# vliu15/speech-masters-thesis

Measured on AMD Instinct MI355X. Metric: LJSpeech utterances/sec per VQ-VAE train step, higher is better.
Workload: dtype bf16

## Files before the change

speech-masters-thesis_amd/csrc/conv_ws.hip:

```cpp
#include <algorithm>
#include <cstdlib>
#include <type_traits>

#include "smt_common.h"
#include "conv_common.h"

namespace smt {

#ifndef SMT_WS_STAMP
#define SMT_WS_STAMP 0
#endif
#if SMT_WS_STAMP
__device__ unsigned long long ws_dbg[256 * 8 * 8];
#define WS_T(var) const unsigned long long var = __builtin_readcyclecounter()
#define WS_ACC(k, a, b) do { if (lane == 0 && wg < 256) ws_dbg[(wg * 8 + wave) * 8 + (k)] += (b) - (a); } while (0)
#else
#define WS_T(var) do {} while (0)
#define WS_ACC(k, a, b) do {} while (0)
#endif
constexpr int WS_AGPR_TAPS = 8;
constexpr int WS_BM = 128, WS_BN = 128, WS_NT = 256, WS_EPI = 128 * 256;
constexpr int WS_KC = 128, WS_ROWB = WS_KC * 2, WS_KSTEPS = WS_KC / 16;

template <int I, int N, typename F>
__device__ __forceinline__ void static_for(F&& f) {
  if constexpr (I < N) {
    f(std::integral_constant<int, I>{});
    static_for<I + 1, N>(f);
  }
}


__device__ __forceinline__ bf16x8 ws_wfrag(const unsigned char* wrow, int kk, int hh, int co) {
  return *reinterpret_cast<const bf16x8*>(wrow + (((2 * kk + hh) ^ (co & 15)) << 4));
}

__device__ __forceinline__ void ws_decode(int tiles_per_batch, int rs, int tile, int& b, int& cls, int& t0) {
  const int bb = tile / tiles_per_batch;
  b = bb / rs; cls = bb - b * rs;
  t0 = (tile - bb * tiles_per_batch) * WS_BM;
}

__device__ __forceinline__ unsigned ws_tap_base(unsigned abase, int ar, int hh) { return abase + ar * WS_ROWB + ((hh ^ swz256_row(ar)) << 4); }
template <int NTAPS>
__device__ __forceinline__ unsigned ws_frag_addr(const unsigned (&tap_base)[NTAPS], int q) {
  return tap_base[q / WS_KSTEPS] ^ (32u * (q % WS_KSTEPS));
}

template <int MW>
__device__ __forceinline__ void ws_read_frags(bf16x8 (&afr)[MW], unsigned ap) {
#pragma unroll
  for (int i = 0; i < MW; ++i)
    asm volatile("ds_read_b128 %0, %1 offset:%2" : "=v"(afr[i]) : "v"(ap), "n"(i * 32 * WS_ROWB));
}
__device__ __forceinline__ void ws_first_use(f32x16& acc) { asm volatile("s_nop 4" : "+v"(acc)); }
__device__ __forceinline__ void ws_first_use(f32x16& acc0, f32x16& acc1) { asm volatile("s_nop 4" : "+v"(acc0), "+v"(acc1)); }
__device__ __forceinline__ void ws_mfma(f32x16& acc, const bf16x8& w, const bf16x8& a, bool w_in_agpr) {
  if (w_in_agpr) asm volatile("v_mfma_f32_32x32x16_bf16 %0, %1, %2, %0" : "+v"(acc) : "a"(w), "v"(a));
  else asm volatile("v_mfma_f32_32x32x16_bf16 %0, %1, %2, %0" : "+v"(acc) : "v"(w), "v"(a));
}
template <int MW>
__device__ __forceinline__ void ws_drain(f32x16 (&acc)[MW]) {
  static_assert(MW == 2 || MW == 4, "the drain names two or four accumulators");
#define WS_DRAIN_NOPS "s_nop 15\n\ts_nop 15\n\ts_nop 15\n\ts_nop 15"
  if constexpr (MW == 4) asm volatile(WS_DRAIN_NOPS : "+v"(acc[0]), "+v"(acc[1]), "+v"(acc[2]), "+v"(acc[3]));
  else asm volatile(WS_DRAIN_NOPS : "+v"(acc[0]), "+v"(acc[1]));
#undef WS_DRAIN_NOPS
}

template <int NTAPS, int MODE>
__global__ __launch_bounds__(WS_NT) void conv_ws_kernel(ConvArgs p, const __bf16* __restrict__ zero_page,
                                                        int tiles_per_wg, int buf_bytes) {
  const bool has_y = MODE == 0 ? (p.y != nullptr) : (MODE == 2);
  const bool has_act_out = MODE == 0 ? (p.act_out != 0) : (MODE == 1);
  const bool has_res = MODE == 0 ? (p.res != nullptr) : (MODE == 2);
  const bool has_epi_act = MODE == 0 ? (p.epi_act != 0) : (MODE == 2);
  typedef __bf16 T;
  constexpr int BM = WS_BM, BN = WS_BN, KC = WS_KC, NT = WS_NT, MW = BM / 32, ROWB = WS_ROWB;
  extern __shared__ __attribute__((aligned(1024))) unsigned char smem[];
  const int tid = threadIdx.x, lane = tid & 63, wave = tid >> 6;
  const int r = lane & 31, hh = lane >> 5;
  const int lrow = lane >> 4, lch = lane & 15;
  const int n0 = blockIdx.y * BN;
  const int rs = p.rs;

  int wg, tile_begin, tile_end;
  if (!wg_tile_run(p.tiles_per_batch * p.B * rs, tiles_per_wg, wg, tile_begin, tile_end)) return;

  unsigned char* lds_res = smem + 2 * (size_t)buf_bytes + wave * (WS_EPI / 4);
  unsigned char* lds_act = lds_res + WS_EPI;
  const unsigned lds_base = (unsigned)(uintptr_t)(__attribute__((address_space(3))) unsigned char*)smem;

  bf16x8 wfrag[NTAPS][KC / 16];
  {
    const int co = n0 + wave * 32 + r;
#pragma unroll
    for (int s = 0; s < NTAPS; ++s) {
      const unsigned char* wrow = reinterpret_cast<const unsigned char*>(p.w) + ((size_t)s * p.Cout + co) * ROWB;
#pragma unroll
      for (int kk = 0; kk < KC / 16; ++kk)
        wfrag[s][kk] = ws_wfrag(wrow, kk, hh, co);
    }
  }
  const int col0 = n0 + wave * 32 + 4 * hh;
  float bval[16];
#pragma unroll
  for (int e = 0; e < 16; ++e) bval[e] = p.bias ? p.bias[col0 + 8 * (e >> 2) + (e & 3)] : 0.f;
  const int rows_in = BM + (NTAPS - 1) * p.dil;
  const int rows_pad = (rows_in + 3) & ~3;

  auto decode = [&](int tile, int& b, int& cls, int& t0) { ws_decode(p.tiles_per_batch, rs, tile, b, cls, t0); };
  const unsigned pitch_x = (unsigned)p.ldx * rs * 2u;
  const unsigned voff_a0 = (unsigned)(4 * wave + lrow) * pitch_x + (unsigned)((lch ^ swz256_row(4 * wave + lrow)) << 4);
  const int ngroups = rows_pad >> 2;
  auto stage_a = [&](int tile, int buf) {
    int b, cls, t0;
    decode(tile, b, cls, t0);
    const int len_full = p.lens_in ? min(scalar_load_i32(p.lens_in + b), p.Tin) : p.Tin;
    const int len_in = max(0, (len_full - cls + rs - 1) / rs);
    const __amdgpu_buffer_rsrc_t rx = ws_rsrc(p.x, ((long long)b * p.x_bs + (long long)cls * p.ldx) * 2, (unsigned)len_in * pitch_x);
    unsigned vo = voff_a0 + (unsigned)(t0 - p.pad) * pitch_x;
    unsigned char* dst = smem + (size_t)buf * buf_bytes + wave * 1024;
    for (int g = wave; g < ngroups; g += NT / 64) {
      ws_dma16(rx, vo, dst);
      vo += 16u * pitch_x; dst += 4096;
    }
  };
  const unsigned echunk = (unsigned)(((lane & 3) ^ ((lane >> 4) & 3)) << 4);
  auto stage_epi = [&](const void* base, long long bs, int ld, int b, int cls, int t0, int Tc, unsigned char* dst) {
    const unsigned pitch = (unsigned)ld * rs * 2u;
    const __amdgpu_buffer_rsrc_t re = ws_rsrc(base, ((long long)b * bs + (long long)cls * ld + n0 + wave * 32) * 2, (unsigned)Tc * pitch);
    unsigned vo = (unsigned)(t0 + (lane >> 2)) * pitch + echunk;
#pragma unroll
    for (int q = 0; q < BM / 16; ++q) {
      ws_dma16(re, vo, dst + q * 1024);
      vo += 16u * pitch;
    }
  };

  stage_a(tile_begin, 0);
  vm_wait<0>();
  for (int tile = tile_begin; tile < tile_end; ++tile) {
    const int buf = (tile - tile_begin) & 1;
    int b, cls, t0;
    decode(tile, b, cls, t0);
    const int Tc = (p.Tout - cls + rs - 1) / rs;
    WS_T(c0);
    __syncthreads();
    WS_T(c1);
    __amdgpu_buffer_rsrc_t rx_n = ws_rsrc(p.x, 0, 0), re_res = rx_n, re_act = rx_n;
    unsigned vo_in = 0, vo_res = 0, vo_act = 0, pitch_res = 0, pitch_act = 0;
    int n_in = 0;
    const int wave_s = __builtin_amdgcn_readfirstlane(wave);
    if constexpr (MODE == 2) {
      if (tile + 1 < tile_end) {
        int nb, ncls, nt0;
        decode(tile + 1, nb, ncls, nt0);
        const int len_full = p.lens_in ? min(scalar_load_i32(p.lens_in + nb), p.Tin) : p.Tin;
        const int len_in = max(0, (len_full - ncls + rs - 1) / rs);
        rx_n = ws_rsrc(p.x, ((long long)nb * p.x_bs + (long long)ncls * p.ldx) * 2, (unsigned)len_in * pitch_x);
        vo_in = voff_a0 + (unsigned)(nt0 - p.pad) * pitch_x;
        n_in = ngroups;
      }
      pitch_res = (unsigned)p.ldr * rs * 2u; pitch_act = (unsigned)p.ldgh * rs * 2u;
      re_res = ws_rsrc(p.res, ((long long)b * p.res_bs + (long long)cls * p.ldr + n0 + wave_s * 32) * 2, (unsigned)Tc * pitch_res);
      re_act = ws_rsrc(p.gate_h, ((long long)b * p.gh_bs + (long long)cls * p.ldgh + n0 + wave_s * 32) * 2, (unsigned)Tc * pitch_act);
      vo_res = (unsigned)(t0 + (lane >> 2)) * pitch_res + echunk;
      vo_act = (unsigned)(t0 + (lane >> 2)) * pitch_act + echunk;
    } else {
      if (tile + 1 < tile_end) stage_a(tile + 1, buf ^ 1);
    }
    WS_T(c2);
    if constexpr (MODE != 2) {
      if (has_res) stage_epi(p.res, p.res_bs, p.ldr, b, cls, t0, Tc, lds_res);
      if (has_epi_act) stage_epi(p.gate_h, p.gh_bs, p.ldgh, b, cls, t0, Tc, lds_act);
    }
    constexpr int WS_EPI_SLOTS = BM / 16, WS_IN_SLOTS = 12, WS_SLOTS = 2 * WS_EPI_SLOTS + WS_IN_SLOTS;
    static_assert(MODE != 2 || WS_SLOTS <= NTAPS * (KC / 16), "one piece per k-step");
    unsigned char* const dst_in = smem + (size_t)(buf ^ 1) * buf_bytes + wave_s * 1024;
    unsigned char* const dst_res = smem + 2 * (size_t)buf_bytes + wave_s * (WS_EPI / 4), * const dst_act = dst_res + WS_EPI;
    auto dma_slot = [&](int s) {
      if (s < WS_EPI_SLOTS) ws_dma16(re_res, vo_res + (unsigned)(16 * s) * pitch_res, dst_res + s * 1024);
      else if (s < 2 * WS_EPI_SLOTS) ws_dma16(re_act, vo_act + (unsigned)(16 * (s - WS_EPI_SLOTS)) * pitch_act, dst_act + (s - WS_EPI_SLOTS) * 1024);
      else {
        const int j = s - 2 * WS_EPI_SLOTS;
        if (wave_s + 4 * j < n_in) ws_dma16(rx_n, vo_in + (unsigned)(16 * j) * pitch_x, dst_in + j * 4096);
      }
    };

    WS_T(c4);
    f32x16 acc[MW];
#pragma unroll
    for (int i = 0; i < MW; ++i)
#pragma unroll
      for (int e = 0; e < 16; ++e) acc[i][e] = 0.f;
    const unsigned abase = lds_base + (unsigned)buf * (unsigned)buf_bytes;
    unsigned tap_base[NTAPS];
#pragma unroll
    for (int s = 0; s < NTAPS; ++s) tap_base[s] = ws_tap_base(abase, r + s * p.dil, hh);
    auto frag_addr = [&](int q) -> unsigned { return ws_frag_addr(tap_base, q); };
    bf16x8 afr[2][MW];
    ws_read_frags(afr[0], frag_addr(0));
#pragma unroll
    for (int q = 0; q < NTAPS * (KC / 16); ++q) {
      if (q + 1 < NTAPS * (KC / 16)) {
        ws_read_frags(afr[(q + 1) & 1], frag_addr(q + 1));
        lgkm_wait<MW>();
      } else {
        lgkm_wait<0>();
      }
#pragma unroll
      for (int i = 0; i < MW; ++i) {
        if (q == 0) ws_first_use(acc[i]);
        ws_mfma(acc[i], wfrag[q / (KC / 16)][q % (KC / 16)], afr[q & 1][i], q / (KC / 16) < WS_AGPR_TAPS);
        if (MODE == 2 && i == 0 && q < WS_SLOTS) {
          __builtin_amdgcn_sched_barrier(0);
          dma_slot(q);
          __builtin_amdgcn_sched_barrier(0);
        }
      }
    }
    ws_drain(acc);
    WS_T(c5);
    vm_wait<0>();
    WS_T(c6);

    const int len_out = p.lens_out ? scalar_load_i32(p.lens_out + b) : 0x7fffffff;
    const unsigned pitch_y = (unsigned)p.ldy * rs * 2u, pitch_u = (unsigned)p.ldya * rs * 2u;
    const __amdgpu_buffer_rsrc_t ry = ws_rsrc(has_y ? p.y : p.x, has_y ? ((long long)b * p.y_bs + (long long)cls * p.ldy + n0 + (MODE == 2 ? wave_s : wave) * 32) * 2 : 0,
                                              has_y ? (unsigned)Tc * pitch_y : 0u);
    const __amdgpu_buffer_rsrc_t ru = ws_rsrc(has_act_out ? p.y_act : p.x,
                                              has_act_out ? ((long long)b * p.ya_bs + (long long)cls * p.ldya + n0 + wave * 32) * 2 : 0,
                                              has_act_out ? (unsigned)Tc * pitch_u : 0u);
    if constexpr (MODE == 2) {
#pragma unroll
      for (int i = 0; i < MW; ++i) {
        const int row = 32 * i + r;
        const int tc = t0 + row;
        const float srow = (cls + rs * tc >= len_out) ? 0.f : p.drop_scale;
        const int swz = (row >> 2) & 3;
        uint2 uv[4], rv[4];
#pragma unroll
        for (int g = 0; g < 4; ++g) {
          const int eoff = row * 64 + ((g ^ swz) << 4) + 8 * hh;
          uv[g] = *reinterpret_cast<const uint2*>(lds_act + eoff);
          rv[g] = *reinterpret_cast<const uint2*>(lds_res + eoff);
        }
        unsigned yp[8];
#pragma unroll
        for (int g = 0; g < 4; ++g) {
          const unsigned uvp[2] = {uv[g].x, uv[g].y}, rvp[2] = {rv[g].x, rv[g].y};
#pragma unroll
          for (int j = 0; j < 2; ++j) {
            const unsigned ypk = pack_bf16x2(acc[i][4 * g + 2 * j] + bval[4 * g + 2 * j], acc[i][4 * g + 2 * j + 1] + bval[4 * g + 2 * j + 1]);
            const float o0 = __builtin_bit_cast(float, ypk << 16), o1 = __builtin_bit_cast(float, ypk & 0xffff0000u);
            const float v0 = (uvp[j] & 0x7fffu) ? o0 * srow : 0.f, v1 = (uvp[j] & 0x7fff0000u) ? o1 * srow : 0.f;
            yp[2 * g + j] = pack_bf16x2(v0 + __builtin_bit_cast(float, rvp[j] << 16), v1 + __builtin_bit_cast(float, rvp[j] & 0xffff0000u));
          }
        }
        pair_up8(yp);
        store_paired(yp, ry, (unsigned)tc * pitch_y + (unsigned)hh * 16u);
      }
    } else {
#pragma unroll
    for (int i = 0; i < MW; ++i) {
      const int row = 32 * i + r;
      const int tc = t0 + row;
      const int ty = cls + rs * tc;
      const float keep_row = (ty >= len_out) ? 0.f : 1.f;
      const int swz = (row >> 2) & 3;
      unsigned yp[8], up[8];
      {
#pragma unroll
      for (int g = 0; g < 4; ++g) {
        float o[4];
#pragma unroll
        for (int k = 0; k < 4; ++k) o[k] = (float)(T)(acc[i][4 * g + k] + bval[4 * g + k]);
        const int eoff = row * 64 + ((g ^ swz) << 4) + 8 * hh;
        if (has_epi_act) {
          const bf16x4 uv = *reinterpret_cast<const bf16x4*>(lds_act + eoff);
#pragma unroll
          for (int k = 0; k < 4; ++k) o[k] = ((float)uv[k] != 0.f) ? o[k] * p.drop_scale : 0.f;
        }
        if (has_res) {
          const bf16x4 rv = *reinterpret_cast<const bf16x4*>(lds_res + eoff);
#pragma unroll
          for (int k = 0; k < 4; ++k) o[k] = fmaf(o[k], keep_row, (float)rv[k]);
        } else {
#pragma unroll
          for (int k = 0; k < 4; ++k) o[k] *= keep_row;
        }
        yp[2 * g] = pack_bf16x2(o[0], o[1]);
        yp[2 * g + 1] = pack_bf16x2(o[2], o[3]);
        if (has_act_out) {
          const int col = col0 + 8 * g;
          const int site = col / p.site_width;
          const unsigned key = site_key(p, site);
          const unsigned long long base = ((unsigned long long)b * p.Ty + ty) * p.site_width + (col - site * p.site_width);
#pragma unroll
          for (int k = 0; k < 4; k += 2) {
            const unsigned h = fmix32((unsigned)((base + k) >> 1) * 0x9E3779B1u + key);
            const bool k0 = (h & 0xFFFFu) >= p.drop_thresh16, k1 = (h >> 16) >= p.drop_thresh16;
            up[2 * g + (k >> 1)] = pack_bf16x2((k0 && o[k] > 0.f) ? o[k] * p.drop_scale : 0.f,
                                               (k1 && o[k + 1] > 0.f) ? o[k + 1] * p.drop_scale : 0.f);
          }
        }
      }
      }
      if (has_y) {
        pair_up8(yp);
        store_paired(yp, ry, (unsigned)tc * pitch_y + (unsigned)hh * 16u);
      }
      if (has_act_out) {
        pair_up8(up);
        store_paired(up, ru, (unsigned)tc * pitch_u + (unsigned)hh * 16u);
      }
    }
    }
    WS_T(c7);
    WS_ACC(0, c0, c1); WS_ACC(1, c1, c2); WS_ACC(3, c2, c4); WS_ACC(4, c4, c5); WS_ACC(5, c5, c6); WS_ACC(6, c6, c7); WS_ACC(7, c0, c0 + 1);
  }
}

template <int NTAPS>
__global__ __launch_bounds__(WS_NT) void conv_ws_pipe_kernel(ConvArgs p, const __bf16* __restrict__ zero_page,
                                                             int tiles_per_wg, int buf_bytes) {
  constexpr int BM = WS_BM, BN = WS_BN, KC = WS_KC, NT = WS_NT, MW = BM / 32, ROWB = WS_ROWB;
  constexpr int NSTEP = NTAPS * (KC / 16), NGAP = NSTEP * MW;
  constexpr int PH_UNIT = 12, PH_ROW = 4 * PH_UNIT + 2, PH_TILE = MW * PH_ROW;
  constexpr int AGPR_TAPS = NTAPS < 8 ? NTAPS : 8;
  static_assert(MW == 4, "four accumulators");
  extern __shared__ __attribute__((aligned(1024))) unsigned char smem[];
  const int tid = threadIdx.x, lane = tid & 63, wave = tid >> 6;
  const int r = lane & 31, hh = lane >> 5;
  const int lrow = lane >> 4, lch = lane & 15;
  const int n0 = blockIdx.y * BN;
  const int rs = p.rs;

  int wg, tile_begin, tile_end;
  if (!wg_tile_run(p.tiles_per_batch * p.B * rs, tiles_per_wg, wg, tile_begin, tile_end)) return;
  const unsigned lds_base = (unsigned)(uintptr_t)(__attribute__((address_space(3))) unsigned char*)smem;

  bf16x8 wfrag[NTAPS][KC / 16];
  {
    const int co = n0 + wave * 32 + r;
#pragma unroll
    for (int s = 0; s < NTAPS; ++s) {
      const unsigned char* wrow = reinterpret_cast<const unsigned char*>(p.w) + ((size_t)s * p.Cout + co) * ROWB;
#pragma unroll
      for (int kk = 0; kk < KC / 16; ++kk)
        wfrag[s][kk] = ws_wfrag(wrow, kk, hh, co);
    }
  }
  const int col0 = n0 + wave * 32 + 4 * hh;
  float bval[16];
#pragma unroll
  for (int e = 0; e < 16; ++e) bval[e] = p.bias ? p.bias[col0 + 8 * (e >> 2) + (e & 3)] : 0.f;
  unsigned keyg[4], cshalf[4];
#pragma unroll
  for (int g = 0; g < 4; ++g) {
    const int col = col0 + 8 * g;
    const int site = col / p.site_width;
    keyg[g] = site_key(p, site);
    cshalf[g] = (unsigned)(col - site * p.site_width) >> 1;
  }
  const int rows_in = BM + (NTAPS - 1) * p.dil;
  const int rows_pad = (rows_in + 3) & ~3;

  auto decode = [&](int tile, int& b, int& cls, int& t0) { ws_decode(p.tiles_per_batch, rs, tile, b, cls, t0); };
  const unsigned pitch_x = (unsigned)p.ldx * rs * 2u;
  const unsigned voff_a0 = (unsigned)(4 * wave + lrow) * pitch_x + (unsigned)((lch ^ swz256_row(4 * wave + lrow)) << 4);
  const int ngroups = rows_pad >> 2;
  auto stage_a = [&](int tile, int buf) {
    int b, cls, t0;
    decode(tile, b, cls, t0);
    const int len_full = p.lens_in ? min(scalar_load_i32(p.lens_in + b), p.Tin) : p.Tin;
    const int len_in = max(0, (len_full - cls + rs - 1) / rs);
    const __amdgpu_buffer_rsrc_t rx = ws_rsrc(p.x, ((long long)b * p.x_bs + (long long)cls * p.ldx) * 2, (unsigned)len_in * pitch_x);
    unsigned vo = voff_a0 + (unsigned)(t0 - p.pad) * pitch_x;
    unsigned char* dst = smem + (size_t)buf * buf_bytes + wave * 1024;
    for (int g = wave; g < ngroups; g += NT / 64) {
      ws_dma16(rx, vo, dst);
      vo += 16u * pitch_x; dst += 4096;
    }
  };

  unsigned pc[MW][8];
  int p_b = 0, p_cls = 0, p_t0 = 0, p_Tc = 0, p_len = 0;
  __amdgpu_buffer_rsrc_t p_ru = ws_rsrc(p.y_act, 0, 0);
  float o0 = 0.f, o1 = 0.f, o2 = 0.f, o3 = 0.f, u0 = 0.f, u1 = 0.f, u2 = 0.f, u3 = 0.f, keepf = 1.f;
  unsigned h0 = 0, h1 = 0, rh = 0, up[8];
  int ty = 0;
  auto fbits = [](unsigned v) { return __builtin_bit_cast(float, v); };
  auto epi = [&](auto M) {
    constexpr int m = decltype(M)::value;
    constexpr int i = m / PH_ROW, rem = m % PH_ROW;
    if constexpr (rem < 4 * PH_UNIT) {
      constexpr int g = rem / PH_UNIT, ph = rem % PH_UNIT;
      if constexpr (ph == 0) {
        if constexpr (g == 0) {
          const int tc = p_t0 + 32 * i + r;
          ty = (tc < p_Tc) ? p_cls + rs * tc : -1;
          keepf = (ty >= p_len) ? 0.f : 1.f;
          rh = (unsigned)((((unsigned long long)p_b * p.Ty + (unsigned)max(ty, 0)) * (unsigned)p.site_width) >> 1);
        }
      } else if constexpr (ph == 1) {
        o0 = fbits(pc[i][2 * g] << 16) * keepf; o1 = fbits(pc[i][2 * g] & 0xffff0000u) * keepf;
      } else if constexpr (ph == 2) {
        o2 = fbits(pc[i][2 * g + 1] << 16) * keepf; o3 = fbits(pc[i][2 * g + 1] & 0xffff0000u) * keepf;
      } else if constexpr (ph == 3) {
        h0 = (rh + cshalf[g]) * 0x9E3779B1u + keyg[g]; h1 = h0 + 0x9E3779B1u;
      } else if constexpr (ph == 4) {
        h0 ^= h0 >> 16; h0 *= 0x85EBCA6Bu; h1 ^= h1 >> 16; h1 *= 0x85EBCA6Bu;
      } else if constexpr (ph == 5) {
        h0 ^= h0 >> 13; h0 *= 0xC2B2AE35u; h1 ^= h1 >> 13; h1 *= 0xC2B2AE35u;
      } else if constexpr (ph == 6) {
        h0 ^= h0 >> 16; h1 ^= h1 >> 16;
      } else if constexpr (ph == 7) {
        u0 = ((h0 & 0xFFFFu) >= p.drop_thresh16 && o0 > 0.f) ? o0 * p.drop_scale : 0.f;
      } else if constexpr (ph == 8) {
        u1 = ((h0 >> 16) >= p.drop_thresh16 && o1 > 0.f) ? o1 * p.drop_scale : 0.f;
      } else if constexpr (ph == 9) {
        u2 = ((h1 & 0xFFFFu) >= p.drop_thresh16 && o2 > 0.f) ? o2 * p.drop_scale : 0.f;
      } else if constexpr (ph == 10) {
        u3 = ((h1 >> 16) >= p.drop_thresh16 && o3 > 0.f) ? o3 * p.drop_scale : 0.f;
      } else {
        up[2 * g] = pack_bf16x2(u0, u1); up[2 * g + 1] = pack_bf16x2(u2, u3);
      }
    } else if constexpr (rem == 4 * PH_UNIT) {
      pair_up8(up);
    } else {
      if (ty >= 0) {
        store_paired(up, p_ru, (unsigned)ty * ((unsigned)p.ldya * 2u) + (unsigned)hh * 16u);
      }
    }
  };

  stage_a(tile_begin, 0);
  vm_wait<0>();
  const int wave_s = __builtin_amdgcn_readfirstlane(wave);
#pragma unroll
  for (int i = 0; i < MW; ++i)
#pragma unroll
    for (int e = 0; e < 8; ++e) pc[i][e] = 0;
  for (int tile = tile_begin; tile < tile_end; ++tile) {
    const int buf = (tile - tile_begin) & 1;
    int b, cls, t0;
    decode(tile, b, cls, t0);
    WS_T(c0);
    __syncthreads();
    WS_T(c1);
    __amdgpu_buffer_rsrc_t rx_n = ws_rsrc(p.x, 0, 0);
    unsigned vo_in = 0;
    int n_in = 0;
    if (tile + 1 < tile_end) {
      int nb, ncls, nt0;
      decode(tile + 1, nb, ncls, nt0);
      const int len_full = p.lens_in ? min(scalar_load_i32(p.lens_in + nb), p.Tin) : p.Tin;
      const int len_in = max(0, (len_full - ncls + rs - 1) / rs);
      rx_n = ws_rsrc(p.x, ((long long)nb * p.x_bs + (long long)ncls * p.ldx) * 2, (unsigned)len_in * pitch_x);
      vo_in = voff_a0 + (unsigned)(nt0 - p.pad) * pitch_x;
      n_in = ngroups;
    }
    unsigned char* const dst_in = smem + (size_t)(buf ^ 1) * buf_bytes + wave_s * 1024;
    constexpr int WS_IN_SLOTS = 12, WS_IN_EVERY = 2;
    static_assert(WS_IN_SLOTS * WS_IN_EVERY <= NSTEP, "the pieces fit the tap loop");
    WS_T(c2);

    f32x16 acc[MW];
#pragma unroll
    for (int i = 0; i < MW; ++i)
#pragma unroll
      for (int e = 0; e < 16; ++e) acc[i][e] = 0.f;
    const unsigned abase = lds_base + (unsigned)buf * (unsigned)buf_bytes;
    unsigned tap_base[NTAPS];
#pragma unroll
    for (int s = 0; s < NTAPS; ++s) tap_base[s] = ws_tap_base(abase, r + s * p.dil, hh);
    auto frag_addr = [&](int q) -> unsigned { return ws_frag_addr(tap_base, q); };
    bf16x8 afr[2][MW];

    ws_read_frags(afr[0], frag_addr(0));
    static_for<0, NSTEP>([&](auto Q) {
      constexpr int q = decltype(Q)::value;
      if constexpr (q + 1 < NSTEP) {
        ws_read_frags(afr[(q + 1) & 1], frag_addr(q + 1));
        lgkm_wait<MW>();
      } else {
        lgkm_wait<0>();
      }
      static_for<0, MW>([&](auto I) {
        constexpr int i = decltype(I)::value;
        if constexpr (q == 0) ws_first_use(acc[i]);
        ws_mfma(acc[i], wfrag[q / (KC / 16)][q % (KC / 16)], afr[q & 1][i], q / (KC / 16) < AGPR_TAPS);
        if constexpr (i == 0 && q % WS_IN_EVERY == 0 && q / WS_IN_EVERY < WS_IN_SLOTS) {
          constexpr int j = q / WS_IN_EVERY;
          __builtin_amdgcn_sched_barrier(0);
          if (wave_s + 4 * j < n_in) ws_dma16(rx_n, vo_in + (unsigned)(16 * j) * pitch_x, dst_in + j * 4096);
          __builtin_amdgcn_sched_barrier(0);
        }
        if constexpr (4 * q + i < PH_TILE) {
          __builtin_amdgcn_sched_barrier(0);
          epi(std::integral_constant<int, 4 * q + i>{});
          __builtin_amdgcn_sched_barrier(0);
        }
      });
    });
    static_for<(NGAP < PH_TILE ? NGAP : PH_TILE), PH_TILE>(epi);
    ws_drain(acc);
    WS_T(c5);
    vm_wait<0>();
    WS_T(c6);
#pragma unroll
    for (int i = 0; i < MW; ++i)
#pragma unroll
      for (int e = 0; e < 16; e += 2) pc[i][e >> 1] = pack_bf16x2(acc[i][e] + bval[e], acc[i][e + 1] + bval[e + 1]);
    p_b = b; p_cls = cls; p_t0 = t0;
    p_ru = ws_rsrc(p.y_act, ((long long)b * p.ya_bs + n0 + wave_s * 32) * 2, (unsigned)p.Ty * ((unsigned)p.ldya * 2u));
    p_Tc = (p.Tout - cls + rs - 1) / rs;
    p_len = p.lens_out ? scalar_load_i32(p.lens_out + b) : 0x7fffffff;
    WS_T(c7);
    WS_ACC(0, c0, c1); WS_ACC(1, c1, c2); WS_ACC(4, c2, c5); WS_ACC(5, c5, c6); WS_ACC(6, c6, c7); WS_ACC(7, c0, c0 + 1);
  }
  static_for<0, PH_TILE>(epi);
}

constexpr int WS2_NT = 512;
constexpr int WS2_MAX_TAPS = 3;

template <int NTAPS, int MODE>
__global__ __launch_bounds__(WS2_NT) void conv_ws2_kernel(ConvArgs p, const __bf16* __restrict__ zero_page,
                                                          int tiles_per_wg, int buf_bytes) {
  constexpr int BM = WS_BM, BN = WS_BN, KC = WS_KC, MW = 2, ROWB = WS_ROWB;
  constexpr int NSTEP = NTAPS * (KC / 16), NG = 5;
  static_assert(MODE == 1 || MODE == 2, "two epilogues");
  constexpr int AGPR_TAPS = NTAPS < 4 ? NTAPS : 4;
  static_assert(NTAPS <= 5, "weights of more than five taps do not fit two waves per SIMD");
  extern __shared__ __attribute__((aligned(1024))) unsigned char smem[];
  const int tid = threadIdx.x, lane = tid & 63;
  const int wave = __builtin_amdgcn_readfirstlane(tid >> 6);
  const int cw = wave & 3, rhalf = wave >> 2;
  const int r = lane & 31, hh = lane >> 5;
  const int n0 = blockIdx.y * BN;
  const int rs = p.rs;

  int wg, tile_begin, tile_end;
  if (!wg_tile_run(p.tiles_per_batch * p.B * rs, tiles_per_wg, wg, tile_begin, tile_end)) return;

  float* lds_bias = reinterpret_cast<float*>(smem + 2 * (size_t)buf_bytes);
  unsigned char* lds_res = smem + 2 * (size_t)buf_bytes + 1024 + wave * (WS_EPI / 8);
  unsigned char* lds_act = lds_res + WS_EPI;
  const unsigned lds_base = (unsigned)(uintptr_t)(__attribute__((address_space(3))) unsigned char*)smem;
  if (tid < BN) lds_bias[tid] = p.bias ? p.bias[n0 + tid] : 0.f;

  bf16x8 wfrag[NTAPS][KC / 16];
  {
    const int co = n0 + cw * 32 + r;
#pragma unroll
    for (int s = 0; s < NTAPS; ++s) {
      const unsigned char* wrow = reinterpret_cast<const unsigned char*>(p.w) + ((size_t)s * p.Cout + co) * ROWB;
#pragma unroll
      for (int kk = 0; kk < KC / 16; ++kk)
        wfrag[s][kk] = ws_wfrag(wrow, kk, hh, co);
    }
  }
  const int col0 = n0 + cw * 32 + 4 * hh;
  const unsigned HC = 0x9E3779B1u;
  const unsigned swh = (unsigned)p.site_width >> 1;
  unsigned kc[4];
  unsigned rowh_lane = 0;
  const unsigned thr_m1 = (p.drop_thresh16 - 1u) * 0x00010001u;
  if (MODE == 1) {
#pragma unroll
    for (int g = 0; g < 4; ++g) {
      const int col = col0 + 8 * g;
      const int site = col / p.site_width;
      kc[g] = ((unsigned)(col - site * p.site_width) >> 1) * HC + site_key(p, site);
    }
    rowh_lane = HC * swh * (unsigned)(rs * r);
  }
  const int rows_in = BM + (NTAPS - 1) * p.dil;
  const int ngroups = (rows_in + 3) >> 2;

  const unsigned pitch_x = (unsigned)p.ldx * rs * 2u;
  unsigned voff_a[NG];
#pragma unroll
  for (int j = 0; j < NG; ++j) {
    const int row = 4 * (wave + 8 * j) + (lane >> 4);
    voff_a[j] = (unsigned)row * pitch_x + (unsigned)(((lane & 15) ^ swz256_row(row)) << 4);
  }
  const unsigned pitch_o = (MODE == 2 ? (unsigned)p.ldy : (unsigned)p.ldya) * rs * 2u;
  const unsigned voff_o = (unsigned)(64 * rhalf + r) * pitch_o + (unsigned)hh * 16u;
  const unsigned pitch_r = (unsigned)p.ldr * rs * 2u, pitch_g = (unsigned)p.ldgh * rs * 2u;
  const int elr = 64 * rhalf + (lane >> 2);
  const unsigned echunk = (unsigned)(((lane & 3) ^ ((lane >> 4) & 3)) << 4);

  auto decode = [&](int tile, int& b, int& cls, int& t0) { ws_decode(p.tiles_per_batch, rs, tile, b, cls, t0); };
  auto stage_a = [&](int tile, int buf) {
    int b, cls, t0;
    decode(tile, b, cls, t0);
    const int len_full = p.lens_in ? min(scalar_load_i32(p.lens_in + b), p.Tin) : p.Tin;
    const int len_in = max(0, (len_full - cls + rs - 1) / rs);
    const __amdgpu_buffer_rsrc_t rx = ws_rsrc(p.x, ((long long)b * p.x_bs + (long long)cls * p.ldx) * 2, (unsigned)len_in * pitch_x);
    const unsigned s0 = (unsigned)(t0 - p.pad) * pitch_x;
    unsigned char* dst = smem + (size_t)buf * buf_bytes + wave * 1024;
#pragma unroll
    for (int j = 0; j < NG; ++j)
      if (wave + 8 * j < ngroups) ws_dma16(rx, voff_a[j] + s0, dst + j * 8192);
  };
  auto stage_epi = [&](const void* base, long long bs, int ld, unsigned pitch, int b, int cls, int t0, int Tc, unsigned char* dst) {
    const __amdgpu_buffer_rsrc_t re = ws_rsrc(base, ((long long)b * bs + (long long)cls * ld + n0 + cw * 32) * 2, (unsigned)Tc * pitch);
#pragma unroll
    for (int q = 0; q < 4; ++q) ws_dma16(re, (unsigned)(t0 + elr + 16 * q) * pitch + echunk, dst + q * 1024);
  };

  f32x16 acc[MW];
  auto epilogue = [&](int b, int cls, int t0, int Tc) {
    const int len_out = p.lens_out ? scalar_load_i32(p.lens_out + b) : 0x7fffffff;
    const __amdgpu_buffer_rsrc_t ry =
        MODE == 2 ? ws_rsrc(p.y, ((long long)b * p.y_bs + (long long)cls * p.ldy + n0 + cw * 32) * 2, (unsigned)Tc * pitch_o)
                  : ws_rsrc(p.y_act, ((long long)b * p.ya_bs + (long long)cls * p.ldya + n0 + cw * 32) * 2, (unsigned)Tc * pitch_o);
    const unsigned so = (unsigned)t0 * pitch_o;
    const unsigned rowh_s = MODE == 1 ? HC * swh * ((unsigned)b * (unsigned)p.Ty + (unsigned)cls + (unsigned)rs * (unsigned)(t0 + 64 * rhalf)) : 0u;
#pragma unroll
    for (int i = 0; i < MW; ++i) {
      const int lr = 32 * i + r;
      const int ty = cls + rs * (t0 + 64 * rhalf + lr);
      const float srow = (ty >= len_out) ? 0.f : p.drop_scale;
      const int swz = (lr >> 2) & 3;
      unsigned yp[8];
      const unsigned rowh = rowh_s + rowh_lane + HC * swh * (unsigned)(rs * 32 * i);
#pragma unroll
      for (int g = 0; g < 4; ++g) {
        const f32x4 bv = *reinterpret_cast<const f32x4*>(lds_bias + cw * 32 + 4 * hh + 8 * g);
        unsigned uvp[2] = {0, 0}, rvp[2] = {0, 0};
        if (MODE == 2) {
          const int eoff = lr * 64 + ((g ^ swz) << 4) + 8 * hh;
          const uint2 uv = *reinterpret_cast<const uint2*>(lds_act + eoff);
          const uint2 rv = *reinterpret_cast<const uint2*>(lds_res + eoff);
          uvp[0] = uv.x; uvp[1] = uv.y; rvp[0] = rv.x; rvp[1] = rv.y;
        }
#pragma unroll
        for (int j = 0; j < 2; ++j) {
          const unsigned ypk = pack_bf16x2(acc[i][4 * g + 2 * j] + bv[2 * j], acc[i][4 * g + 2 * j + 1] + bv[2 * j + 1]);
          const float o0 = __builtin_bit_cast(float, ypk << 16), o1 = __builtin_bit_cast(float, ypk & 0xffff0000u);
          if (MODE == 1) {
            unsigned w = pk_relu_bf16(pack_bf16x2(o0 * srow, o1 * srow));
            if (p.drop_thresh16) w &= pk_keep_mask(fmix32(rowh + kc[g] + (unsigned)j * HC), thr_m1);
            yp[2 * g + j] = w;
          } else {
            const unsigned u2 = uvp[j], r2 = rvp[j];
            const float v0 = (u2 & 0x7fffu) ? o0 * srow : 0.f, v1 = (u2 & 0x7fff0000u) ? o1 * srow : 0.f;
            yp[2 * g + j] = pack_bf16x2(v0 + __builtin_bit_cast(float, r2 << 16), v1 + __builtin_bit_cast(float, r2 & 0xffff0000u));
          }
        }
      }
#pragma unroll
      for (int h2 = 0; h2 < 2; ++h2)
#pragma unroll
        for (int d = 0; d < 2; ++d) {
          auto sw = __builtin_amdgcn_permlane32_swap(yp[4 * h2 + d], yp[4 * h2 + 2 + d], false, false);
          yp[4 * h2 + d] = sw[0]; yp[4 * h2 + 2 + d] = sw[1];
        }
      store_paired(yp, ry, voff_o + so + (unsigned)(32 * i) * pitch_o);
    }
  };

  stage_a(tile_begin, 0);
  vm_wait<0>();
  int pb = 0, pcls = 0, pt0 = 0, pTc = 0;
  for (int tile = tile_begin; tile < tile_end; ++tile) {
    const int buf = (tile - tile_begin) & 1;
    int b, cls, t0;
    decode(tile, b, cls, t0);
    const int Tc = (p.Tout - cls + rs - 1) / rs;
    WS_T(c0);
    __syncthreads();
    WS_T(c1);
    if (tile + 1 < tile_end) stage_a(tile + 1, buf ^ 1);
    WS_T(c2);
    if (rhalf == 1 && tile > tile_begin) epilogue(pb, pcls, pt0, pTc);
    WS_T(c3);
    if (MODE == 2) {
      stage_epi(p.res, p.res_bs, p.ldr, pitch_r, b, cls, t0, Tc, lds_res);
      stage_epi(p.gate_h, p.gh_bs, p.ldgh, pitch_g, b, cls, t0, Tc, lds_act);
    }
    WS_T(c4);
#pragma unroll
    for (int i = 0; i < MW; ++i)
#pragma unroll
      for (int e = 0; e < 16; ++e) acc[i][e] = 0.f;
    const unsigned abase = lds_base + (unsigned)buf * (unsigned)buf_bytes + (unsigned)(64 * rhalf) * ROWB;
    unsigned tap_base[NTAPS];
#pragma unroll
    for (int s = 0; s < NTAPS; ++s) {
      const int ar = r + s * p.dil;
      tap_base[s] = abase + ar * ROWB + ((hh ^ swz256_row(ar)) << 4);
    }
    auto frag_addr = [&](int q) -> unsigned { return ws_frag_addr(tap_base, q); };
    bf16x8 afr[3][MW];
#pragma unroll
    for (int q0 = 0; q0 < 2; ++q0) {
      const unsigned ap = frag_addr(q0);
      ws_read_frags(afr[q0], ap);
    }
    static_for<0, NSTEP>([&](auto Q) {
      constexpr int q = decltype(Q)::value;
      if constexpr (q + 2 < NSTEP) {
        const unsigned ap = frag_addr(q + 2);
        ws_read_frags(afr[(q + 2) % 3], ap);
        lgkm_wait<2 * MW>();
      } else if constexpr (q + 1 < NSTEP) {
        lgkm_wait<MW>();
      } else {
        lgkm_wait<0>();
      }
      static_assert(MW == 2, "two accumulators per wave");
      if constexpr (q == 0) ws_first_use(acc[0], acc[1]);
      ws_mfma(acc[0], wfrag[q / (KC / 16)][q % (KC / 16)], afr[q % 3][0], q / (KC / 16) < AGPR_TAPS);
      ws_mfma(acc[1], wfrag[q / (KC / 16)][q % (KC / 16)], afr[q % 3][1], q / (KC / 16) < AGPR_TAPS);
    });
    ws_drain(acc);
    WS_T(c5);
    vm_wait<0>();
    WS_T(c6);
    if (rhalf == 0) epilogue(b, cls, t0, Tc);
    WS_T(c7);
    WS_ACC(0, c0, c1); WS_ACC(1, c1, c2); WS_ACC(2, c2, c3); WS_ACC(3, c3, c4); WS_ACC(4, c4, c5); WS_ACC(5, c5, c6);
    WS_ACC(6, c6, c7); WS_ACC(7, c0, c0 + 1);
    pb = b; pcls = cls; pt0 = t0; pTc = Tc;
  }
  if (rhalf == 1) epilogue(pb, pcls, pt0, pTc);
}

#ifndef SMT_WS_AB
#define SMT_WS_AB 0
#endif

static int ws_min_tiles() {
  static const int v = getenv("SMT_WS_MIN_TILES") ? atoi(getenv("SMT_WS_MIN_TILES")) : 512;
  return v;
}

bool plan_conv_ws(ConvArgs& p, WsPlan& pl) {
  static const bool no_ws = getenv("SMT_CONV_NO_WS") != nullptr;
  const int tc_max = (p.Tout + p.rs - 1) / p.rs;
  const int rows_pad = (WS_BM + (p.taps - 1) * p.dil + 3) & ~3;
  const int buf_bytes = (int)align_up((size_t)std::max(rows_pad * 256, WS_BM * (WS_BN + 8) * 2), 1024);
  const size_t lds = 2 * (size_t)buf_bytes + 2 * WS_EPI;
  const int tpb = (tc_max + WS_BM - 1) / WS_BM;
  const long long ntiles = (long long)tpb * p.B * p.rs;
  if (no_ws || p.Cin != 128 || p.taps < 3 || p.taps > 9 || !(p.taps & 1) || lds > 160 * 1024 || ntiles < ws_min_tiles()) return false;
  p.tiles_per_batch = tpb;
  const int nwg = 256;
  pl.buf_bytes = buf_bytes; pl.lds = lds;
  pl.tiles_per_wg = (int)((ntiles + nwg - 1) / nwg);
  pl.grid = dim3((unsigned)nwg, (unsigned)(p.Cout / WS_BN));
  return true;
}

enum WsVariant { WS2_FWD, WS2_DGRAD, WS_PIPE, WS_MODE1, WS_MODE2, WS_GENERIC };
static WsVariant ws_variant(const ConvArgs& p) {
  const bool y = p.y != nullptr, ao = p.act_out != 0, res = p.res != nullptr, ea = p.epi_act != 0;
  const bool fwd = !y && ao && !res && !ea, dgrad = y && !ao && res && ea;
#if SMT_WS_AB
  static const bool no_ws2 = getenv("SMT_CONV_NO_WS2") != nullptr, no_pipe = getenv("SMT_CONV_NO_PIPE") != nullptr;
#else
  constexpr bool no_ws2 = false, no_pipe = false;
#endif
  if (p.taps <= WS2_MAX_TAPS && !no_ws2 && (fwd || dgrad)) return fwd ? WS2_FWD : WS2_DGRAD;
  if (fwd) return no_pipe ? WS_MODE1 : WS_PIPE;
  return dgrad ? WS_MODE2 : WS_GENERIC;
}

const char* conv_ws_variant_name(const ConvArgs& p) {
  switch (ws_variant(p)) {
    case WS2_FWD: case WS2_DGRAD: return "conv_ws2";
    case WS_PIPE: return "conv_ws_pipe";
    default: return "conv_ws";
  }
}

template <typename K>
static void launch_ws_kernel(K kernel, int nt, size_t lds, const ConvArgs& p, const WsPlan& pl, const void* zero_page, hipStream_t stream) {
  (void)hipFuncSetAttribute((const void*)kernel, hipFuncAttributeMaxDynamicSharedMemorySize, 160 * 1024);
  kernel<<<pl.grid, nt, lds, stream>>>(p, (const __bf16*)zero_page, pl.tiles_per_wg, pl.buf_bytes);
}

template <int NTAPS>
static void launch_ws(const ConvArgs& p, const WsPlan& pl, const void* zero_page, hipStream_t stream) {
  constexpr bool ws2 = NTAPS <= WS2_MAX_TAPS, one_wave = SMT_WS_AB || !ws2;
  const WsVariant v = ws_variant(p);
  if constexpr (ws2) {
    if (v == WS2_FWD) return launch_ws_kernel(conv_ws2_kernel<NTAPS, 1>, WS2_NT, 2 * (size_t)pl.buf_bytes + 1024, p, pl, zero_page, stream);
    if (v == WS2_DGRAD) return launch_ws_kernel(conv_ws2_kernel<NTAPS, 2>, WS2_NT, pl.lds + 1024, p, pl, zero_page, stream);
  }
  if constexpr (one_wave) {
    if (v == WS_PIPE) return launch_ws_kernel(conv_ws_pipe_kernel<NTAPS>, WS_NT, pl.lds, p, pl, zero_page, stream);
    if (v == WS_MODE2) return launch_ws_kernel(conv_ws_kernel<NTAPS, 2>, WS_NT, pl.lds, p, pl, zero_page, stream);
  }
  if constexpr (SMT_WS_AB) {
    if (v == WS_MODE1) return launch_ws_kernel(conv_ws_kernel<NTAPS, 1>, WS_NT, pl.lds, p, pl, zero_page, stream);
  }
  launch_ws_kernel(conv_ws_kernel<NTAPS, 0>, WS_NT, pl.lds, p, pl, zero_page, stream);
}

void launch_conv_ws(const ConvArgs& p, const WsPlan& pl, const void* zero_page, hipStream_t stream) {
  switch (p.taps) {
    case 3: return launch_ws<3>(p, pl, zero_page, stream);
    case 5: return launch_ws<5>(p, pl, zero_page, stream);
    case 7: return launch_ws<7>(p, pl, zero_page, stream);
    default: return launch_ws<9>(p, pl, zero_page, stream);
  }
}

}

using namespace smt;

#if SMT_WS_STAMP
extern "C" int smt_ws_debug_dump(unsigned long long* host, int n, int reset) {
  int rc = (int)hipMemcpyFromSymbol(host, HIP_SYMBOL(ws_dbg), sizeof(unsigned long long) * n);
  if (reset) { static unsigned long long z[256 * 8 * 8]; rc |= (int)hipMemcpyToSymbol(HIP_SYMBOL(ws_dbg), z, sizeof(z)); }
  return rc;
}
#endif
```

Baseline: 526.0.

## Restructure interleaved dropout-ReLU epilogue with cheaper hashing and packed mask ops

Rewrites the epilogue that is interleaved with the MFMA loop in the pipelined conv kernel. The per-row hash base is folded into precomputed constants (row and lane increments, a combined column key), and the threshold test becomes a packed saturating-subtract mask. ReLU and scaling are applied on packed bf16 pairs instead of through scalar compare-selects. Epilogue phases are remapped so they skip the MFMA slots that issue DMA and the early fragment reads. This should cut VALU work and register pressure inside the MFMA shadow, at the risk of hash or rounding mismatches, for example when the unsigned products wrap or when rows past the valid range are padding.

```diff
diff --git a/speech-masters-thesis_amd/csrc/conv_ws.hip b/speech-masters-thesis_amd/csrc/conv_ws.hip
--- a/speech-masters-thesis_amd/csrc/conv_ws.hip
+++ b/speech-masters-thesis_amd/csrc/conv_ws.hip
@@ -327,7 +327,7 @@
                                                              int tiles_per_wg, int buf_bytes) {
   constexpr int BM = WS_BM, BN = WS_BN, KC = WS_KC, NT = WS_NT, MW = BM / 32, ROWB = WS_ROWB;
   constexpr int NSTEP = NTAPS * (KC / 16), NGAP = NSTEP * MW;
-  constexpr int PH_UNIT = 12, PH_ROW = 4 * PH_UNIT + 2, PH_TILE = MW * PH_ROW;
+  constexpr int PH_PAIR = 5, PH_ROW = 2 + 8 * PH_PAIR + 2, PH_TILE = MW * PH_ROW;
   constexpr int AGPR_TAPS = NTAPS < 8 ? NTAPS : 8;
   static_assert(MW == 4, "four accumulators");
   extern __shared__ __attribute__((aligned(1024))) unsigned char smem[];
@@ -356,14 +356,19 @@
   float bval[16];
 #pragma unroll
   for (int e = 0; e < 16; ++e) bval[e] = p.bias ? p.bias[col0 + 8 * (e >> 2) + (e & 3)] : 0.f;
-  unsigned keyg[4], cshalf[4];
+  const unsigned HC = 0x9E3779B1u;
+  const unsigned swh = (unsigned)p.site_width >> 1;
+  unsigned kc[4];
 #pragma unroll
   for (int g = 0; g < 4; ++g) {
     const int col = col0 + 8 * g;
     const int site = col / p.site_width;
-    keyg[g] = site_key(p, site);
-    cshalf[g] = (unsigned)(col - site * p.site_width) >> 1;
-  }
+    kc[g] = ((unsigned)(col - site * p.site_width) >> 1) * HC + site_key(p, site);
+  }
+  const unsigned rowh_lane = HC * swh * (unsigned)(rs * r);
+  const unsigned rowh_step = HC * swh * (unsigned)(rs * 32);
+  const unsigned thr_m1 = (p.drop_thresh16 - 1u) * 0x00010001u;
+  const unsigned keep_all = p.drop_thresh16 ? 0u : 0xffffffffu;
   const int rows_in = BM + (NTAPS - 1) * p.dil;
   const int rows_pad = (rows_in + 3) & ~3;
 
@@ -386,49 +391,58 @@
   };
 
   unsigned pc[MW][8];
-  int p_b = 0, p_cls = 0, p_t0 = 0, p_Tc = 0, p_len = 0;
+  int p_cls = 0, p_t0 = 0, p_Tc = 0, p_len = 0;
+  unsigned p_rowh = 0;
   __amdgpu_buffer_rsrc_t p_ru = ws_rsrc(p.y_act, 0, 0);
-  float o0 = 0.f, o1 = 0.f, o2 = 0.f, o3 = 0.f, u0 = 0.f, u1 = 0.f, u2 = 0.f, u3 = 0.f, keepf = 1.f;
-  unsigned h0 = 0, h1 = 0, rh = 0, up[8];
+  float o0 = 0.f, o1 = 0.f, srow = 0.f;
+  unsigned h = 0, mk = 0, rowh = 0, up[8];
   int ty = 0;
   auto fbits = [](unsigned v) { return __builtin_bit_cast(float, v); };
+  auto pin = [](auto& v) { asm volatile("" : "+v"(v)); };
+  unsigned one2 = 0x00010001u;
+  asm volatile("" : "+s"(one2));
   auto epi = [&](auto M) {
     constexpr int m = decltype(M)::value;
     constexpr int i = m / PH_ROW, rem = m % PH_ROW;
-    if constexpr (rem < 4 * PH_UNIT) {
-      constexpr int g = rem / PH_UNIT, ph = rem % PH_UNIT;
+    if constexpr (rem == 0) {
+      const int tc = p_t0 + 32 * i + r;
+      ty = (tc < p_Tc) ? p_cls + rs * tc : -1;
+      pin(ty);
+    } else if constexpr (rem == 1) {
+      srow = (ty >= p_len) ? 0.f : p.drop_scale;
+      rowh = p_rowh + (unsigned)i * rowh_step + rowh_lane;
+      pin(srow); pin(rowh);
+    } else if constexpr (rem < 2 + 8 * PH_PAIR) {
+      constexpr int pr = (rem - 2) / PH_PAIR, ph = (rem - 2) % PH_PAIR, g = pr >> 1, j = pr & 1;
       if constexpr (ph == 0) {
-        if constexpr (g == 0) {
-          const int tc = p_t0 + 32 * i + r;
-          ty = (tc < p_Tc) ? p_cls + rs * tc : -1;
-          keepf = (ty >= p_len) ? 0.f : 1.f;
-          rh = (unsigned)((((unsigned long long)p_b * p.Ty + (unsigned)max(ty, 0)) * (unsigned)p.site_width) >> 1);
-        }
+        h = rowh + kc[g] + (unsigned)j * HC; h ^= h >> 16; h *= 0x85EBCA6Bu;
+        pin(h);
       } else if constexpr (ph == 1) {
-        o0 = fbits(pc[i][2 * g] << 16) * keepf; o1 = fbits(pc[i][2 * g] & 0xffff0000u) * keepf;
+        h ^= h >> 13; h *= 0xC2B2AE35u;
+        pin(h);
       } else if constexpr (ph == 2) {
-        o2 = fbits(pc[i][2 * g + 1] << 16) * keepf; o3 = fbits(pc[i][2 * g + 1] & 0xffff0000u) * keepf;
+        h ^= h >> 16;
+        u16x2v d = __builtin_elementwise_sub_sat(__builtin_bit_cast(u16x2v, h), __builtin_bit_cast(u16x2v, thr_m1));
+        pin(d);
+        d = __builtin_elementwise_min(d, __builtin_bit_cast(u16x2v, one2));
+        mk = __builtin_bit_cast(unsigned, (u16x2v)(u16x2v{0, 0} - d));
+        pin(mk);
       } else if constexpr (ph == 3) {
-        h0 = (rh + cshalf[g]) * 0x9E3779B1u + keyg[g]; h1 = h0 + 0x9E3779B1u;
-      } else if constexpr (ph == 4) {
-        h0 ^= h0 >> 16; h0 *= 0x85EBCA6Bu; h1 ^= h1 >> 16; h1 *= 0x85EBCA6Bu;
-      } else if constexpr (ph == 5) {
-        h0 ^= h0 >> 13; h0 *= 0xC2B2AE35u; h1 ^= h1 >> 13; h1 *= 0xC2B2AE35u;
-      } else if constexpr (ph == 6) {
-        h0 ^= h0 >> 16; h1 ^= h1 >> 16;
-      } else if constexpr (ph == 7) {
-        u0 = ((h0 & 0xFFFFu) >= p.drop_thresh16 && o0 > 0.f) ? o0 * p.drop_scale : 0.f;
-      } else if constexpr (ph == 8) {
-        u1 = ((h0 >> 16) >= p.drop_thresh16 && o1 > 0.f) ? o1 * p.drop_scale : 0.f;
-      } else if constexpr (ph == 9) {
-        u2 = ((h1 & 0xFFFFu) >= p.drop_thresh16 && o2 > 0.f) ? o2 * p.drop_scale : 0.f;
-      } else if constexpr (ph == 10) {
-        u3 = ((h1 >> 16) >= p.drop_thresh16 && o3 > 0.f) ? o3 * p.drop_scale : 0.f;
+        o0 = fbits(pc[i][pr] << 16) * srow;
+        pin(o0);
+        o1 = fbits(pc[i][pr] & 0xffff0000u) * srow;
+        pin(o1);
       } else {
-        up[2 * g] = pack_bf16x2(u0, u1); up[2 * g + 1] = pack_bf16x2(u2, u3);
-      }
-    } else if constexpr (rem == 4 * PH_UNIT) {
+        typedef float f32x2 __attribute__((ext_vector_type(2)));
+        typedef __bf16 bf16x2 __attribute__((ext_vector_type(2)));
+        const unsigned w = __builtin_bit_cast(unsigned, __builtin_convertvector((f32x2){o0, o1}, bf16x2));
+        up[pr] = pk_relu_bf16(w) & (mk | keep_all);
+        pin(up[pr]);
+      }
+    } else if constexpr (rem == 2 + 8 * PH_PAIR) {
       pair_up8(up);
+#pragma unroll
+      for (int e = 0; e < 8; ++e) pin(up[e]);
     } else {
       if (ty >= 0) {
         store_paired(up, p_ru, (unsigned)ty * ((unsigned)p.ldya * 2u) + (unsigned)hh * 16u);
@@ -498,14 +512,19 @@
           if (wave_s + 4 * j < n_in) ws_dma16(rx_n, vo_in + (unsigned)(16 * j) * pitch_x, dst_in + j * 4096);
           __builtin_amdgcn_sched_barrier(0);
         }
-        if constexpr (4 * q + i < PH_TILE) {
+        constexpr bool dma_gap = i == 0 && q % WS_IN_EVERY == 0 && q / WS_IN_EVERY < WS_IN_SLOTS;
+        constexpr int dma_gaps_before = std::min((q + WS_IN_EVERY - 1) / WS_IN_EVERY, WS_IN_SLOTS) + (i > 0 && q % WS_IN_EVERY == 0 && q / WS_IN_EVERY < WS_IN_SLOTS ? 1 : 0);
+        constexpr int READ_SKIP = std::max(0, std::min(NSTEP - 1, NGAP - WS_IN_SLOTS - PH_TILE));
+        constexpr bool read_gap = i == MW - 1 && q < READ_SKIP;
+        constexpr int m = MW * q + i - dma_gaps_before - std::min(q, READ_SKIP);
+        if constexpr (!dma_gap && !read_gap && m < PH_TILE) {
           __builtin_amdgcn_sched_barrier(0);
-          epi(std::integral_constant<int, 4 * q + i>{});
+          epi(std::integral_constant<int, m>{});
           __builtin_amdgcn_sched_barrier(0);
         }
       });
     });
-    static_for<(NGAP < PH_TILE ? NGAP : PH_TILE), PH_TILE>(epi);
+    static_for<std::min(NGAP - WS_IN_SLOTS, PH_TILE), PH_TILE>(epi);
     ws_drain(acc);
     WS_T(c5);
     vm_wait<0>();
@@ -514,7 +533,8 @@
     for (int i = 0; i < MW; ++i)
 #pragma unroll
       for (int e = 0; e < 16; e += 2) pc[i][e >> 1] = pack_bf16x2(acc[i][e] + bval[e], acc[i][e + 1] + bval[e + 1]);
-    p_b = b; p_cls = cls; p_t0 = t0;
+    p_cls = cls; p_t0 = t0;
+    p_rowh = HC * swh * ((unsigned)b * (unsigned)p.Ty + (unsigned)cls + (unsigned)rs * (unsigned)t0);
     p_ru = ws_rsrc(p.y_act, ((long long)b * p.ya_bs + n0 + wave_s * 32) * 2, (unsigned)p.Ty * ((unsigned)p.ldya * 2u));
     p_Tc = (p.Tout - cls + rs - 1) / rs;
     p_len = p.lens_out ? scalar_load_i32(p.lens_out + b) : 0x7fffffff;
```

Result: faster. 537.2, median of 4 (+2.1%).
